# jianzhnie/ScaleRL

Hardware: NVIDIA H100
Metric: learner_frames_per_sec (higher is better)
Workload: dtype bf16

## Files before the change

### scalerl_b200/csrc/encoder.cu

```cuda
#include "encoder_problems.cuh"
#include "tma_problems.cuh"
#include "res_problems.cuh"
#include "enc_fused.cuh"
#include "kernels.h"
#include <stdio.h>
#include <stdlib.h>

namespace srl {

constexpr int PACK_BLOCKS_FK = 256, PACK_BLOCKS_FD = 256, PACK_BLOCKS_CONV = 288;
SRL_DEVINL void pack_store(bf16* __restrict__ out, bf16* __restrict__ out_lo, int64_t i, float v) {
  const bf16 hi = __float2bfloat16_rn(v);
  out[i] = hi;
  if (out_lo) out_lo[i] = __float2bfloat16_rn(v - __bfloat162float(hi));
}
SRL_DEVINL void pack_store2(bf16* __restrict__ out, bf16* __restrict__ out_lo, int64_t i, float v0, float v1) {
  const bf16 h0 = __float2bfloat16_rn(v0), h1 = __float2bfloat16_rn(v1);
  *reinterpret_cast<uint32_t*>(out + i) = pack_bf16x2(v0, v1);
  if (out_lo) *reinterpret_cast<uint32_t*>(out_lo + i) = pack_bf16x2(v0 - __bfloat162float(h0), v1 - __bfloat162float(h1));
}
__global__ void __launch_bounds__(256) pack_weights_kernel(ParamPtrs p, bf16* __restrict__ out, bf16* __restrict__ out_lo, int skip_w1k) {
  pdl_wait(2);
  __shared__ __align__(16) float tile[64 * 99];
  const int t = threadIdx.x, b = blockIdx.x;
  if (b < PACK_BLOCKS_FK) {
    const float4* src = reinterpret_cast<const float4*>(p.wf + (size_t)(2 * b) * 3136);
    float4 v[7];
#pragma unroll
    for (int u = 0; u < 7; ++u) { const int q = t + 256 * u; if (q < 1568) v[u] = __ldg(src + q); }
#pragma unroll
    for (int u = 0; u < 7; ++u) { const int q = t + 256 * u; if (q < 1568) *reinterpret_cast<float4*>(tile + 4 * q) = v[u]; }
    __syncthreads();
#pragma unroll 4
    for (int pp = t; pp < 2 * 1568; pp += 256) {
      const int r = pp >= 1568, k = 2 * (pp - r * 1568), hw = k >> 6, c = k & 63;
      const float* row = tile + r * 3136;
      pack_store2(out, out_lo, WPack::WFK + (int64_t)(2 * b + r) * 3136 + k, row[c * 49 + hw], row[(c + 1) * 49 + hw]);
    }
  } else if (b < PACK_BLOCKS_FK + PACK_BLOCKS_FD) {
    const int bb = b - PACK_BLOCKS_FK, j0 = (bb & 7) * 64, c0 = (bb >> 3) * 2;
    float2 v[13];
#pragma unroll
    for (int u = 0; u < 13; ++u) {
      const int q = t + 256 * u, jj = q / 49, e = q - jj * 49;
      if (q < 64 * 49) v[u] = __ldg(reinterpret_cast<const float2*>(p.wf + (size_t)(j0 + jj) * 3136 + c0 * 49 + 2 * e));
    }
#pragma unroll
    for (int u = 0; u < 13; ++u) {
      const int q = t + 256 * u, jj = q / 49, e = q - jj * 49;
      if (q < 64 * 49) { tile[jj * 99 + 2 * e] = v[u].x; tile[jj * 99 + 2 * e + 1] = v[u].y; }
    }
    __syncthreads();
    const int lane = t & 31, warp = t >> 5;
    for (int kk = warp; kk < 98; kk += 8) {
      const int cc = kk >= 49, hw = kk - cc * 49;
      pack_store2(out, out_lo, WPack::WFD + (int64_t)(hw * 64 + c0 + cc) * 512 + j0 + 2 * lane, tile[(2 * lane) * 99 + kk], tile[(2 * lane + 1) * 99 + kk]);
    }
  } else {
    const int bb = b - PACK_BLOCKS_FK - PACK_BLOCKS_FD;
    constexpr int64_t NCONV = WPack::WFK + (WPack::TOTAL - WPack::W3D);
    for (int64_t n = (int64_t)bb * 256 + t; n < NCONV; n += (int64_t)PACK_BLOCKS_CONV * 256) {
      const int64_t i = n < WPack::WFK ? n : n - WPack::WFK + WPack::W3D;
      float v;
      if (i < WPack::W2K) {
        if (skip_w1k) continue;
        const int e = (int)(i - WPack::W1K), co = e >> 8, k = e & 255, tap = k >> 6, q = k & 63;
        const int c = q >> 4, dy = (q >> 2) & 3, dx = q & 3, kh = 4 * (tap >> 1) + dy, kw = 4 * (tap & 1) + dx;
        v = p.w1[co * 256 + c * 64 + kh * 8 + kw];
      } else if (i < WPack::W3K) {
        const int e = (int)(i - WPack::W2K), co = e >> 9, k = e & 511, tap = k >> 5, c = k & 31;
        v = p.w2[((co * 32 + c) << 4) + tap];
      } else if (i < WPack::WFK) {
        const int e = (int)(i - WPack::W3K), co = e / 576, k = e - co * 576, tap = k >> 6, c = k & 63;
        v = p.w3[(co * 64 + c) * 9 + tap];
      } else if (i < WPack::W2D) {
        const int e = (int)(i - WPack::W3D), c = e / 576, k = e - c * 576, tap = k >> 6, co = k & 63;
        v = p.w3[(co * 64 + c) * 9 + tap];
      } else {
        const int e = (int)(i - WPack::W2D), cls = e >> 13, r = e & 8191, c = r >> 8, k = r & 255, tt = k >> 6, co = k & 63;
        const int kh = (cls >> 1) + 2 * (tt >> 1), kw = (cls & 1) + 2 * (tt & 1);
        v = p.w2[((co * 32 + c) << 4) + kh * 4 + kw];
      }
      pack_store(out, out_lo, i, v);
    }
  }
}

__global__ void __launch_bounds__(352) obs_s2d_kernel(const uint8_t* __restrict__ obs, bf16* __restrict__ xs, int frame_blocks,
                                                      const float* __restrict__ w1, bf16* __restrict__ w1k, bf16* __restrict__ w1k_lo) {
  pdl_wait(1);
  pdl_launch();
  if ((int)blockIdx.x >= frame_blocks) {
    const int e = ((int)blockIdx.x - frame_blocks) * 352 + (int)threadIdx.x;
    if (e < 32 * 256 && w1k) {
      const int co = e >> 8, k = e & 255, tap = k >> 6, q = k & 63;
      const int c = q >> 4, dy = (q >> 2) & 3, dx = q & 3, kh = 4 * (tap >> 1) + dy, kw = 4 * (tap & 1) + dx;
      pack_store(w1k, w1k_lo, e, __ldg(w1 + co * 256 + c * 64 + kh * 8 + kw));
    }
    return;
  }
  __shared__ uint32_t tile[21][16][21];
  const int n = blockIdx.x;
  const int t = threadIdx.x;
  if (t < 336) {
    const int g = t / 21, X = t - g * 21;
    const uint8_t* src = obs + (size_t)n * 28224 + (g >> 2) * 7056 + (g & 3) * 84;
#pragma unroll
    for (int y = 0; y < 21; ++y) tile[y][g][X] = __ldg(reinterpret_cast<const uint32_t*>(src + y * 336) + X);
  }
  __syncthreads();
  if (t < 336) {
    const int X = t >> 4, g = t & 15;
#pragma unroll
    for (int y = 0; y < 21; ++y) {
      const uint32_t w = tile[y][g][X];
      const float f0 = __uint_as_float(__byte_perm(w, 0x4B000000u, 0x7540)) - 8388608.f;
      const float f1 = __uint_as_float(__byte_perm(w, 0x4B000000u, 0x7541)) - 8388608.f;
      const float f2 = __uint_as_float(__byte_perm(w, 0x4B000000u, 0x7542)) - 8388608.f;
      const float f3 = __uint_as_float(__byte_perm(w, 0x4B000000u, 0x7543)) - 8388608.f;
      *reinterpret_cast<uint2*>(xs + (((size_t)n * 21 + y) * 21 + X) * 64 + g * 4) = make_uint2(pack_bf16x2(f0, f1), pack_bf16x2(f2, f3));
    }
  }
}

__global__ void __launch_bounds__(256) a3_transpose_kernel(const bf16* __restrict__ a3, bf16* __restrict__ a3t) {
  pdl_wait(53);
  __shared__ __align__(16) uint16_t tile[49 * 66];
  const int n = blockIdx.x, t = threadIdx.x;
  const uint4* src = reinterpret_cast<const uint4*>(a3 + (size_t)n * 3136);
  for (int q = t; q < 392; q += 256) {
    const uint4 v = __ldg(src + q);
    uint32_t* d = reinterpret_cast<uint32_t*>(tile + (q >> 3) * 66 + (q & 7) * 8);
    d[0] = v.x; d[1] = v.y; d[2] = v.z; d[3] = v.w;
  }
  __syncthreads();
  uint32_t* dst = reinterpret_cast<uint32_t*>(a3t + (size_t)n * 3136);
  for (int pp = t; pp < 1568; pp += 256) {
    const int o = 2 * pp, c0 = o / 49, h0 = o - c0 * 49, o1 = o + 1, c1 = o1 / 49, h1 = o1 - c1 * 49;
    dst[pp] = (uint32_t)tile[h0 * 66 + c0] | ((uint32_t)tile[h1 * 66 + c1] << 16);
  }
}
SRL_KSTAMP_SETTER(kstamp_set_encoder)

cudaError_t launch_a3_transpose(const bf16* a3, bf16* a3t, int frames, cudaStream_t st) {
  if (frames <= 0) return cudaSuccess;
  a3_transpose_kernel<<<frames, 256, 0, st>>>(a3, a3t);
  return cudaGetLastError();
}

cudaError_t launch_pack_weights(const ParamPtrs& p, bf16* wpack, cudaStream_t st, bf16* wpack_lo, bool skip_w1k) {
  pack_weights_kernel<<<PACK_BLOCKS_FK + PACK_BLOCKS_FD + PACK_BLOCKS_CONV, 256, 0, st>>>(p, wpack, wpack_lo, skip_w1k ? 1 : 0);
  return cudaGetLastError();
}

#define SRL_TRY(x) do { cudaError_t e_ = (x); if (e_ != cudaSuccess) return e_; } while (0)

static inline int cdiv(int a, int b) { return (a + b - 1) / b; }

typedef CUresult (*EncodeTiledFn)(CUtensorMap*, CUtensorMapDataType, cuuint32_t, void*, const cuuint64_t*, const cuuint64_t*,
                                  const cuuint32_t*, const cuuint32_t*, CUtensorMapInterleave, CUtensorMapSwizzle,
                                  CUtensorMapL2promotion, CUtensorMapFloatOOBfill);

static EncodeTiledFn encode_fn() {
  static EncodeTiledFn fn = nullptr;
  if (!fn) {
    void* f = nullptr;
    cudaDriverEntryPointQueryResult q;
    if (cudaGetDriverEntryPoint("cuTensorMapEncodeTiled", &f, cudaEnableDefault, &q) == cudaSuccess && q == cudaDriverEntryPointSuccess)
      fn = reinterpret_cast<EncodeTiledFn>(f);
  }
  return fn;
}

bool make_map(CUtensorMap* m, const void* base, int rank, const uint64_t* dims, const uint64_t* strides_elems, const uint32_t* box,
              bool swizzle64) {
  EncodeTiledFn fn = encode_fn();
  if (!fn) return false;
  cuuint64_t gd[5], gs[4];
  cuuint32_t bx[5], es[5];
  for (int i = 0; i < rank; ++i) { gd[i] = dims[i]; bx[i] = box[i]; es[i] = 1; }
  for (int i = 0; i + 1 < rank; ++i) gs[i] = strides_elems[i] * 2;
  return fn(m, CU_TENSOR_MAP_DATA_TYPE_BFLOAT16, (cuuint32_t)rank, const_cast<void*>(base), gd, gs, bx, es, CU_TENSOR_MAP_INTERLEAVE_NONE,
            swizzle64 ? CU_TENSOR_MAP_SWIZZLE_64B : CU_TENSOR_MAP_SWIZZLE_128B, CU_TENSOR_MAP_L2_PROMOTION_L2_128B,
            CU_TENSOR_MAP_FLOAT_OOB_FILL_NONE) == CUDA_SUCCESS;
}

struct MapBuilder {
  const char* failed = nullptr;
  bool lo = false, failed_lo = false;
  void operator()(CUtensorMap* m, const void* base, uint64_t inner, uint64_t rows, uint32_t box_inner, uint32_t box_rows, const char* name,
                  bool swizzle64 = false) {
    const uint64_t d[2] = {inner, rows}, s[1] = {inner};
    const uint32_t bx[2] = {box_inner, box_rows};
    if (!failed && !make_map(m, base, 2, d, s, bx, swizzle64)) { failed = name; failed_lo = lo; }
  }
};

static void build_operand_maps(MapBuilder& mk, const OperandTensors& b, uint64_t nf, uint64_t nb, OperandMaps* M) {
  mk(&M->a1p0_w, b.a1, 64, nf * 100, 64, RConv2Fwd::WROWS, "a1p0_w");
  mk(&M->a1p1_w, b.a1 + (size_t)nf * 100 * 64, 64, nf * 100, 64, RConv2Fwd::WROWS, "a1p1_w");
  mk(&M->a2_w, b.a2, 64, nf * 81, 64, RConv3Fwd::WROWS, "a2_w");
  mk(&M->da3g_w, b.da3, 64, nb * 81, 64, RConv3Dgrad::WROWS, "da3g_w");
  mk(&M->da3g_b, b.da3, 64, nb * 81, 64, 128, "da3g_b");
  mk(&M->da2g_w, b.da2, 64, nb * 100, 64, RConv2Dgrad::WROWS, "da2g_w");
  mk(&M->da2g_b, b.da2, 64, nb * 100, 64, 128, "da2g_b");
  mk(&M->da1g_b, b.da1, 32, nb * 441, 32, 128, "da1g_b", true);
  mk(&M->a3m128, b.a3, 3136, nf, 64, 128, "a3m128");
  mk(&M->a3m64, b.a3, 3136, nf, 64, 64, "a3m64");
  mk(&M->dhm128, b.dh, 512, nb, 64, 128, "dhm128");
  mk(&M->dhm64, b.dh, 512, nb, 64, 64, "dhm64");
  const bf16* w = b.wpack;
  mk(&M->w1k, w + WPack::W1K, 256, 32, 64, 32, "w1k");
  mk(&M->w2k, w + WPack::W2K, 512, 64, 64, 64, "w2k");
  mk(&M->w3k, w + WPack::W3K, 576, 64, 64, 64, "w3k");
  mk(&M->wfk, w + WPack::WFK, 3136, 512, 64, 64, "wfk");
  mk(&M->wfd, w + WPack::WFD, 512, 3136, 64, 64, "wfd");
  mk(&M->w3d, w + WPack::W3D, 576, 64, 64, 64, "w3d");
  mk(&M->w2d, w + WPack::W2D, 256, 128, 64, 128, "w2d");
}

cudaError_t build_tma_maps(const EncoderBuffers& b, int NF, int NB, TmaMaps* M, const char** why) {
  static_assert(RConv1Wgrad::WROWS == RConv1Fwd::WROWS && RConv2Wgrad::WROWS == RConv2Fwd::WROWS && RConv3Wgrad::WROWS == RConv3Fwd::WROWS,
                "forward and wgrad share the window maps");
  const uint64_t nf = NF, nb = NB;
  MapBuilder mk;
  mk(&M->xs_w, b.xs, 64, nf * 441, 64, RConv1Fwd::WROWS, "xs_w");
  mk(&M->a3tm64, b.a3t, 3136, nf, 64, 64, "a3tm64");
  build_operand_maps(mk, b.hi, nf, nb, &M->hi);
  mk.lo = true;
  if (b.lo.wpack) build_operand_maps(mk, b.lo, nf, nb, &M->lo);
  M->valid = !mk.failed;
  if (mk.failed && why) {
    static thread_local char name[32];
    snprintf(name, sizeof(name), "%s%s", mk.failed, mk.failed_lo ? "_lo" : "");
    *why = name;
  }
  return mk.failed ? cudaErrorInvalidValue : cudaSuccess;
}

static cudaError_t launch_s2d(const uint8_t* obs, int frames, bf16* xs, cudaStream_t st, const float* w1, bf16* w1k, bf16* w1k_lo) {
  constexpr int WB = (32 * 256 + 351) / 352;
  SRL_TRY(launch_chain(obs_s2d_kernel, dim3(frames + WB), dim3(352), 0, st, obs, xs, frames, w1, w1k, w1k_lo));
  return cudaGetLastError();
}

static int sm_count() {
  static const int n = [] { int d = 0, v = 0; cudaGetDevice(&d); cudaDeviceGetAttribute(&v, cudaDevAttrMultiProcessorCount, d); return v > 0 ? v : 132; }();
  return n;
}
static int persistent_ctas() {
  static int v = 0;
  if (!v) {
    const char* e = getenv("SRL_PERSISTENT_CTAS");
    v = e ? atoi(e) : sm_count();
    if (v < 16 || v > sm_count()) v = sm_count();
  }
  return v;
}
#define kPersistentCtas persistent_ctas()
static int bwd_ctas() {
  static const int v = [] { const char* e = getenv("SRL_BWD_CTAS"); int x = e ? atoi(e) : 0; return x < 16 || x > sm_count() ? 0 : x; }();
  return v ? v : persistent_ctas() - persistent_ctas() / 9;
}
static int side_wgrad_ctas() {
  static const int v = [] { const char* e = getenv("SRL_WGRAD_CTAS"); int x = e ? atoi(e) : 64; return x < 8 || x > sm_count() ? 64 : x; }();
  return v;
}

struct WgradReduce3 {
  static constexpr int KID = 0, CO = 64, BIAS = 64, PART = WSP_W3, NR = 18, ROW_GROUPS = 32;
  static constexpr bool FRAMES_U8 = false;
  SRL_DEVINL static int row(int rg, int i) { return (i % 9) * 64 + 2 * rg + i / 9; }
};
struct WgradReduce2 {
  static constexpr int KID = 0, CO = 64, BIAS = 64, PART = WSP_W2, NR = 16, ROW_GROUPS = 32;
  static constexpr bool FRAMES_U8 = false;
  SRL_DEVINL static int row(int rg, int i) { return (i >> 2) * 128 + (i & 3) * 32 + rg; }
};
struct WgradReduce1 {
  static constexpr int KID = 51, CO = 32, BIAS = 32, PART = WSP_W1, NR = 16, ROW_GROUPS = 16;
  static constexpr bool FRAMES_U8 = true;
  SRL_DEVINL static int row(int rg, int i) {
    const int c = rg >> 2, kh2 = (rg >> 1) & 1, dy = 2 * (rg & 1) + (i >> 3), kw = i & 7;
    return kh2 * 128 + (kw >> 2) * 64 + c * 16 + dy * 4 + (kw & 3);
  }
};
template <class L>
__global__ void __launch_bounds__(L::NR * 8) conv_wgrad_reduce_kernel(const float* __restrict__ part, int n, float* __restrict__ g,
                                                                       float* __restrict__ db) {
  constexpr int CG = L::CO / 8, TILES = L::ROW_GROUPS * CG;
  static_assert(L::BIAS <= 8 * L::NR, "the bias block fits the tile's threads and shared memory");
  extern __shared__ __align__(16) float stage[];
  pdl_wait(L::KID);
  pdl_launch();
  const int t = threadIdx.x, rg = blockIdx.x / CG, co0 = (blockIdx.x % CG) * 8;
  const bool bias = blockIdx.x == TILES;
  const int per = bias ? L::BIAS / 4 : 2 * L::NR;
  for (int k = t; k < n * per; k += L::NR * 8) {
    const int c = k / per, q = k - c * per;
    const float* src = part + (size_t)c * L::PART + (bias ? L::PART - L::BIAS + 4 * q : L::row(rg, q >> 1) * L::CO + co0 + 4 * (q & 1));
    asm volatile("cp.async.cg.shared.global [%0], [%1], 16;" ::"r"(smem_u32(stage + 4 * k)), "l"(src) : "memory");
  }
  asm volatile("cp.async.wait_all;" ::: "memory");
  __syncthreads();
  const int w = bias ? L::BIAS : 8 * L::NR;
  if (t >= w) return;
  float s = 0.f;
  for (int c = 0; c < n; ++c) s += stage[c * w + t];
  if (bias) db[t] += s;
  else g[(size_t)(co0 + (t & 7)) * (L::ROW_GROUPS * L::NR) + L::NR * rg + (t >> 3)] = L::FRAMES_U8 ? s * (1.0f / 255.0f) : s;
}

template <class L>
static cudaError_t launch_wgrad_reduce(const float* part, int n, float* g, float* db, cudaStream_t st) {
  static PerDeviceOnce once;
  SRL_TRY(ensure_max_dynamic_smem(once, conv_wgrad_reduce_kernel<L>, WG_PART_CTAS * L::NR * 32));
  static const int greatest = [] { int lo = 0, hi = 0; return cudaDeviceGetStreamPriorityRange(&lo, &hi) == cudaSuccess ? hi : 0; }();
  cudaLaunchConfig_t cfg = {};
  cfg.gridDim = dim3(L::ROW_GROUPS * (L::CO / 8) + 1); cfg.blockDim = dim3(L::NR * 8); cfg.dynamicSmemBytes = (size_t)n * L::NR * 32; cfg.stream = st;
  cudaLaunchAttribute attr[1];
  attr[0].id = cudaLaunchAttributePriority;
  attr[0].val.priority = greatest;
  cfg.attrs = attr; cfg.numAttrs = 1;
  return cudaLaunchKernelEx(&cfg, conv_wgrad_reduce_kernel<L>, part, n, g, db);
}

cudaError_t encoder_forward(const uint8_t* obs, int frames, const ParamPtrs& p, const EncoderBuffers& buf, const TmaMaps& maps, int mode,
                            const StepStreams& S, bool fused_front) {
  if (frames <= 0) return cudaSuccess;
  if ((mode != 0 && mode != 1) || !maps.valid) return cudaErrorInvalidValue;
  const int sp = mode;
  if (sp && !buf.lo.wpack) return cudaErrorInvalidValue;
  const cudaStream_t st = S.main;
  if (fused_front && !sp && (reinterpret_cast<uintptr_t>(obs) & 15) == 0) {
    EncFusedParams q{obs, p.w1, p.b1, p.w2, p.b2, buf.xs, buf.hi.a1, buf.hi.a2, frames, buf.NF};
    S.b(PS_ENC_FUSED); SRL_TRY(enc_fused_fwd_launch(q, kPersistentCtas, st)); S.e(PS_ENC_FUSED);
    SRL_TRY(S.join(LANE_PACK));
  } else {
  S.b(PS_S2D); SRL_TRY(launch_s2d(obs, frames, buf.xs, st, p.w1, buf.hi.wpack + WPack::W1K, sp ? buf.lo.wpack + WPack::W1K : nullptr)); S.e(PS_S2D);
  { RConv1Fwd::Params q{maps.xs_w, maps.hi.w1k, maps.lo.w1k, p.b1, buf.hi.a1, buf.lo.a1, frames, buf.NF};
    S.b(PS_CONV1_FWD); SRL_TRY(res_fwd_launch<RConv1Fwd>(q, cdiv(frames * 441, 128), kPersistentCtas, st, sp)); S.e(PS_CONV1_FWD); }
  SRL_TRY(S.join(LANE_PACK));
  { RConv2Fwd::Params q{maps.hi.a1p0_w, maps.hi.a1p1_w, maps.hi.w2k, maps.lo.a1p0_w, maps.lo.a1p1_w, maps.lo.w2k, p.b2, buf.hi.a2, buf.lo.a2, frames};
    S.b(PS_CONV2_FWD); SRL_TRY(res_fwd_launch<RConv2Fwd>(q, cdiv(frames * 100, 128), kPersistentCtas, st, sp)); S.e(PS_CONV2_FWD); }
  }
  { RConv3Fwd::Params q{maps.hi.a2_w, maps.hi.w3k, maps.lo.a2_w, maps.lo.w3k, p.b3, buf.hi.a3, buf.lo.a3, frames};
    S.b(PS_CONV3_FWD); SRL_TRY(res_fwd_launch<RConv3Fwd>(q, cdiv(frames * 81, 128), kPersistentCtas, st, sp)); S.e(PS_CONV3_FWD); }
  { TFcFwd::Params q{maps.hi.a3m128, maps.hi.wfk, maps.lo.a3m128, maps.lo.wfk, buf.hpart, frames};
    static_assert(TFcFwd::SPLITS == FC_SPLITS, "split count");
    S.b(PS_FC_FWD);
    if (sp) SRL_TRY((igemm_tma_launch<TFcFwd, 1>(q, dim3(cdiv(frames, 128), 8 * FC_SPLITS), st)));
    else SRL_TRY((igemm_tma_launch<TFcFwd, 0>(q, dim3(cdiv(frames, 128), 8 * FC_SPLITS), st)));
    S.e(PS_FC_FWD); }
  return cudaSuccess;
}

cudaError_t encoder_backward(int frames, const EncoderBuffers& buf, const ParamPtrs& g, const TmaMaps& maps, int mode,
                             const StepStreams& S, BwdParts parts, bool a3t_done) {
  if (frames <= 0) return cudaSuccess;
  if ((mode != 0 && mode != 1) || !maps.valid) return cudaErrorInvalidValue;
  const int sp = mode;
  if (sp && !buf.lo.wpack) return cudaErrorInvalidValue;
  const bool do_fc = parts & BWD_FC, do_conv = parts & BWD_CONV;
  const cudaStream_t st = S.main, s1 = S.lane(LANE_FC_WGRAD), s2 = S.lane(LANE_CONV3_WGRAD), s3 = S.lane(LANE_CONV2_WGRAD);
  if (do_fc) {
    SRL_TRY(S.fork(LANE_FC_WGRAD));
    { const bool native = !sp && buf.a3t != nullptr;
      S.b(PS_FC_WGRAD);
      if (native) {
        if (!a3t_done) SRL_TRY(launch_a3_transpose(buf.hi.a3, buf.a3t, frames, s1));
        TFcWgradN::Params q{maps.hi.dhm64, maps.a3tm64, g.wf, g.bf, frames};
        SRL_TRY((igemm_tma_launch<TFcWgradN, 0>(q, dim3(1, 4 * (TFcWgradN::NCT + 1)), s1)));
      } else {
        TFcWgrad::Params q{maps.hi.dhm64, maps.hi.a3m64, maps.lo.dhm64, maps.lo.a3m64, g.wf, g.bf, frames};
        if (sp) SRL_TRY((igemm_tma_launch<TFcWgrad, 1>(q, dim3(1, 4 * 50), s1))); else SRL_TRY((igemm_tma_launch<TFcWgrad, 0>(q, dim3(1, 4 * 50), s1)));
      }
      S.e(PS_FC_WGRAD); }
    { TFcDgrad::Params q{maps.hi.dhm128, maps.hi.wfd, maps.lo.dhm128, maps.lo.wfd, buf.hi.a3, buf.hi.da3, buf.lo.da3, frames};
      S.b(PS_FC_DGRAD);
      if (sp) SRL_TRY((igemm_tma_launch<TFcDgrad, 1>(q, dim3(cdiv(frames, 128), 49), st))); else SRL_TRY((igemm_tma_launch<TFcDgrad, 0>(q, dim3(cdiv(frames, 128), 49), st)));
      S.e(PS_FC_DGRAD); }
    if (!do_conv) SRL_TRY(S.join(LANE_FC_WGRAD));
  }
  if (!do_conv) return cudaSuccess;
  SRL_TRY(S.fork(LANE_CONV3_WGRAD));
  float* part3 = buf.wgrad_part;
  float* part2 = part3 + (size_t)WG_PART_CTAS * WSP_W3;
  float* part1 = part2 + (size_t)WG_PART_CTAS * WSP_W2;
  int n3 = 0, n2 = 0, n1 = 0;
  { RConv3Wgrad::Params q{maps.hi.a2_w, maps.hi.da3g_b, maps.lo.a2_w, maps.lo.da3g_b, part3, frames * 81, 0};
    S.b(PS_CONV3_WGRAD); SRL_TRY(res_wgrad_launch<RConv3Wgrad>(q, side_wgrad_ctas(), s2, &n3, sp)); S.e(PS_CONV3_WGRAD); }
  if (!S.collapsed) SRL_TRY(launch_wgrad_reduce<WgradReduce3>(part3, n3, g.w3, g.b3, s2));
  { RConv3Dgrad::Params q{maps.hi.da3g_w, maps.hi.w3d, maps.lo.da3g_w, maps.lo.w3d, buf.hi.a2, buf.hi.da2, buf.lo.da2, frames};
    S.b(PS_CONV3_DGRAD); SRL_TRY(res_fwd_launch<RConv3Dgrad>(q, cdiv(frames * 81, 128), bwd_ctas(), st, sp)); S.e(PS_CONV3_DGRAD); }
  SRL_TRY(S.fork(LANE_CONV2_WGRAD));
  { RConv2Wgrad::Params q{maps.hi.a1p0_w, maps.hi.a1p1_w, maps.hi.da2g_b, maps.lo.a1p0_w, maps.lo.a1p1_w, maps.lo.da2g_b, part2, frames * 100, 0};
    S.b(PS_CONV2_WGRAD); SRL_TRY(res_wgrad_launch<RConv2Wgrad>(q, side_wgrad_ctas(), s3, &n2, sp)); S.e(PS_CONV2_WGRAD); }
  if (!S.collapsed) SRL_TRY(launch_wgrad_reduce<WgradReduce2>(part2, n2, g.w2, g.b2, s3));
  { RConv2Dgrad::Params q{maps.hi.da2g_w, maps.hi.w2d, maps.lo.da2g_w, maps.lo.w2d, buf.hi.a1, buf.hi.da1, buf.lo.da1, frames, buf.NF};
    S.b(PS_CONV2_DGRAD); SRL_TRY(res_fwd_launch<RConv2Dgrad>(q, cdiv(frames * 100, 128), bwd_ctas(), st, sp)); S.e(PS_CONV2_DGRAD); }
  { RConv1Wgrad::Params q{maps.xs_w, maps.hi.da1g_b, maps.lo.da1g_b, part1, frames * 441, 0};
    S.b(PS_CONV1_WGRAD); SRL_TRY(res_wgrad_launch<RConv1Wgrad>(q, bwd_ctas(), st, &n1, sp)); S.e(PS_CONV1_WGRAD); }
  S.b(PS_WGRAD_FINALIZE);
  if (S.collapsed) {
    SRL_TRY(launch_wgrad_reduce<WgradReduce3>(part3, n3, g.w3, g.b3, st));
    SRL_TRY(launch_wgrad_reduce<WgradReduce2>(part2, n2, g.w2, g.b2, st));
  }
  SRL_TRY(launch_wgrad_reduce<WgradReduce1>(part1, n1, g.w1, g.b1, st));
  S.e(PS_WGRAD_FINALIZE);
  if (do_fc) SRL_TRY(S.join(LANE_FC_WGRAD));
  SRL_TRY(S.join(LANE_CONV3_WGRAD));
  SRL_TRY(S.join(LANE_CONV2_WGRAD));
  return cudaSuccess;
}

}
```

### scalerl_b200/csrc/igemm_tma.cuh

```cuda
#pragma once
#include <cuda.h>
#include "common.cuh"
#include "kernels.h"

namespace srl {

SRL_DEVINL void tma_prefetch_desc(const CUtensorMap* m) {
  asm volatile("prefetch.tensormap [%0];" ::"l"(reinterpret_cast<uint64_t>(m)) : "memory");
}
SRL_DEVINL void tma_load_2d(void* dst, const CUtensorMap* m, uint64_t* bar, int c0, int c1) {
  asm volatile("cp.async.bulk.tensor.2d.shared::cluster.global.mbarrier::complete_tx::bytes [%0], [%1, {%3, %4}], [%2];"
               ::"r"(smem_u32(dst)), "l"(reinterpret_cast<uint64_t>(m)), "r"(smem_u32(bar)), "r"(c0), "r"(c1) : "memory");
}
SRL_DEVINL void tma_load_3d(void* dst, const CUtensorMap* m, uint64_t* bar, int c0, int c1, int c2) {
  asm volatile("cp.async.bulk.tensor.3d.shared::cluster.global.mbarrier::complete_tx::bytes [%0], [%1, {%3, %4, %5}], [%2];"
               ::"r"(smem_u32(dst)), "l"(reinterpret_cast<uint64_t>(m)), "r"(smem_u32(bar)), "r"(c0), "r"(c1), "r"(c2) : "memory");
}
SRL_DEVINL void tma_load_4d(void* dst, const CUtensorMap* m, uint64_t* bar, int c0, int c1, int c2, int c3) {
  asm volatile("cp.async.bulk.tensor.4d.shared::cluster.global.mbarrier::complete_tx::bytes [%0], [%1, {%3, %4, %5, %6}], [%2];"
               ::"r"(smem_u32(dst)), "l"(reinterpret_cast<uint64_t>(m)), "r"(smem_u32(bar)), "r"(c0), "r"(c1), "r"(c2), "r"(c3)
               : "memory");
}
SRL_DEVINL void tma_load_5d(void* dst, const CUtensorMap* m, uint64_t* bar, int c0, int c1, int c2, int c3, int c4) {
  asm volatile("cp.async.bulk.tensor.5d.shared::cluster.global.mbarrier::complete_tx::bytes [%0], [%1, {%3, %4, %5, %6, %7}], [%2];"
               ::"r"(smem_u32(dst)), "l"(reinterpret_cast<uint64_t>(m)), "r"(smem_u32(bar)), "r"(c0), "r"(c1), "r"(c2), "r"(c3), "r"(c4)
               : "memory");
}

constexpr int IGT_THREADS = 288;

template <class P, int SPLIT = 0>
struct TmaCfg {
  static constexpr int KROWS = P::A_MN ? P::KROWS : 64;
  static constexpr int A_BYTES = P::A_MN ? 2 * KROWS * 128 : 128 * 128;
  static constexpr int B_BLOCKS = (P::BN + 63) / 64;
  static constexpr int B_BYTES = P::B_MN ? B_BLOCKS * KROWS * 128 : P::BN * 128;
  static constexpr int HALF_BYTES = A_BYTES + B_BYTES;
  static constexpr int STAGE_BYTES = HALF_BYTES * (1 + SPLIT);
  static constexpr int NB = P::BN / 2;
  static constexpr int STAGES = fit_stages(P::STAGES, 2 * WG_IMG_BYTES + 1024 + 256, STAGE_BYTES);
  static constexpr int SMEM_BYTES = STAGES * STAGE_BYTES + 2 * WG_IMG_BYTES + 1024 + 256;
  static_assert(SMEM_BYTES <= 232448, "shared memory budget (227 KB)");
  static_assert(NB == 32 || NB == 64 || NB == 128, "MMA N per warpgroup");
  static constexpr int MMAS = P::A_MN ? KROWS / 16 : 4;
  static_assert(A_BYTES % 1024 == 0 && B_BYTES % 1024 == 0, "operand tiles must keep 1024 B alignment (SWIZZLE_128B atoms)");
  static_assert(P::A_MN == P::B_MN, "mixed majors are not used");
  static_assert(KROWS % 16 == 0, "contraction rows per stage must be a multiple of MMA K = 16");
};

template <class P, int SPLIT>
SRL_DEVINL void igt_epilogue(const typename P::Params& p, int tm, int ty, int row, int c0, float (&v)[16]) {
  if constexpr (SPLIT) P::template epilogue16<1>(p, tm, ty, row, c0, v); else P::epilogue16(p, tm, ty, row, c0, v);
}
template <class P, int SPLIT>
SRL_DEVINL void igt_epilogue(const typename P::Params& p, int tm, int ty, int row, int c0, float (&v)[16], const uint4 (&pre)[2]) {
  if constexpr (SPLIT) P::template epilogue16<1>(p, tm, ty, row, c0, v, pre); else P::epilogue16(p, tm, ty, row, c0, v, pre);
}

template <class P, int SPLIT = 0>
__global__ void __launch_bounds__(IGT_THREADS) igemm_tma_kernel(const __grid_constant__ typename P::Params p) {
  using C = TmaCfg<P, SPLIT>;
  extern __shared__ uint8_t smem_raw[];
  uint8_t* smem = reinterpret_cast<uint8_t*>((reinterpret_cast<uintptr_t>(smem_raw) + 1023) & ~uintptr_t(1023));
  float* img = reinterpret_cast<float*>(smem + C::STAGES * C::STAGE_BYTES);
  uint64_t* bars = reinterpret_cast<uint64_t*>(smem + C::STAGES * C::STAGE_BYTES + 2 * WG_IMG_BYTES);
  uint64_t* full = bars;
  uint64_t* empty = bars + C::STAGES;

  const int tid = threadIdx.x;
  const int warp = tid >> 5;
  const int tm = blockIdx.x, ty = blockIdx.y;
  const int nkb = P::num_kblocks(p, tm, ty);

  if constexpr (P::ZERO_INIT) {
    if (P::zero_cta(ty)) {
      uint4* z = reinterpret_cast<uint4*>(smem);
      for (int i = tid; i < C::STAGES * C::STAGE_BYTES / 16; i += IGT_THREADS) z[i] = make_uint4(0, 0, 0, 0);
    }
    __syncthreads();
    for (int s = 0; s < C::STAGES; ++s) P::init_smem(p, tm, ty, smem + s * C::STAGE_BYTES, tid);
    fence_proxy_async_smem();
  }
  if (warp == 8 && (tid & 31) == 0) {
    for (int s = 0; s < C::STAGES; ++s) { mbar_init(&full[s], 1); mbar_init(&empty[s], 8); }
    mbar_fence_init();
    P::prefetch(p);
  }
  __syncthreads();
  pdl_wait(P::KID);
  if (tid == 256) pdl_launch();

  if (warp == 8) {
    const uint32_t leader = elect_one_sync();
    for (int kb = 0; kb < nkb; ++kb) {
      const int s = kb % C::STAGES;
      mbar_wait(&empty[s], ((kb / C::STAGES) & 1) ^ 1);
      if (leader) {
        uint8_t* sA = smem + s * C::STAGE_BYTES;
        if constexpr (SPLIT) P::issue_split(p, tm, ty, kb, sA, C::A_BYTES, C::HALF_BYTES, &full[s]);
        else P::issue(p, tm, ty, kb, sA, sA + C::A_BYTES, &full[s]);
      }
      __syncwarp();
    }
  } else {
    const int g = warp >> 2, wt = tid & 127;
    constexpr int NB = C::NB;
    uint4 pre[P::PREFETCH ? NB / 16 : 1][2];
    if constexpr (P::PREFETCH) {
#pragma unroll
      for (int c = 0; c < NB / 16; ++c) P::prefetch16(p, tm, ty, wt, g * NB + c * 16, pre[c]);
    }
    float acc[2][NB / 2];
#pragma unroll
    for (int h = 0; h < 2; ++h)
#pragma unroll
      for (int i = 0; i < NB / 2; ++i) acc[h][i] = 0.f;
    constexpr uint32_t ASTEP = P::A_MN ? 2048 / 16 : 32 / 16, BSTEP = P::B_MN ? 2048 / 16 : 32 / 16;
    constexpr uint32_t A_HI = (P::A_MN ? C::KROWS * 128 : 64 * 128) / 16;
    const uint32_t b_off = P::B_MN ? (g * NB / 64) * C::KROWS * 128 + (g * NB % 64) * 2 : g * NB * 128;
    for (int kb = 0; kb < nkb; ++kb) {
      const int s = kb % C::STAGES;
      mbar_wait(&full[s], (kb / C::STAGES) & 1);
      const uint32_t a0 = smem_u32(smem + s * C::STAGE_BYTES);
      const uint64_t ad0 = P::A_MN ? make_smem_desc(a0, C::KROWS * 128, 1024) : make_smem_desc(a0, 16, 1024);
      const uint64_t bd0 = P::B_MN ? make_smem_desc(a0 + C::A_BYTES + b_off, C::KROWS * 128, 1024) : make_smem_desc(a0 + C::A_BYTES + b_off, 16, 1024);
      wg_fence();
#pragma unroll
      for (int k = 0; k < C::MMAS; ++k) {
        const uint64_t ad = ad0 + (uint64_t)(k * ASTEP), bd = bd0 + (uint64_t)(k * BSTEP);
        wg_mma128<NB, P::A_MN ? 1 : 0, P::B_MN ? 1 : 0>(acc, ad, A_HI, bd, (kb | k) != 0);
        if constexpr (SPLIT) {
          wg_mma128<NB, P::A_MN ? 1 : 0, P::B_MN ? 1 : 0>(acc, ad, A_HI, bd + (uint64_t)(C::HALF_BYTES / 16), 1);
          wg_mma128<NB, P::A_MN ? 1 : 0, P::B_MN ? 1 : 0>(acc, ad + (uint64_t)(C::HALF_BYTES / 16), A_HI, bd, 1);
        }
      }
      wg_commit();
      if constexpr (C::STAGES > 1) {
        wg_wait_prev();
        __syncwarp();
        if (kb > 0 && (tid & 31) == 0) mbar_arrive(&empty[(kb - 1) % C::STAGES]);
      } else {
        wg_wait_all();
        __syncwarp();
        if ((tid & 31) == 0) mbar_arrive(&empty[s]);
      }
    }
    wg_wait_all();
    wg_fence_regs(acc[0]); wg_fence_regs(acc[1]);
    float* my_img = img + g * (WG_IMG_BYTES / 4);
#pragma unroll
    for (int c = 0; c < NB / 16; ++c) {
      float v[16];
      wg_acc_row16<NB>(acc, c, my_img, wt, 2 + g, v);
      if constexpr (P::PREFETCH) igt_epilogue<P, SPLIT>(p, tm, ty, wt, g * NB + c * 16, v, pre[c]);
      else igt_epilogue<P, SPLIT>(p, tm, ty, wt, g * NB + c * 16, v);
    }
  }
}

template <class P, int SPLIT = 0>
cudaError_t igemm_tma_launch(const typename P::Params& p, dim3 grid, cudaStream_t stream) {
  using C = TmaCfg<P, SPLIT>;
  if (grid.x == 0 || grid.y == 0) return cudaSuccess;
  static PerDeviceOnce once;
  { cudaError_t e = ensure_max_dynamic_smem(once, igemm_tma_kernel<P, SPLIT>, C::SMEM_BYTES); if (e != cudaSuccess) return e; }
  return launch_chain(igemm_tma_kernel<P, SPLIT>, grid, dim3(IGT_THREADS), C::SMEM_BYTES, stream, p);
}

}
```

### scalerl_b200/csrc/tma_problems.cuh

```cuda
#pragma once
#include "igemm_tma.cuh"
#include "encoder_problems.cuh"

namespace srl {

#define SRL_TMAP alignas(64) CUtensorMap

struct TFcFwd {
  static constexpr int KID = 31;
  static constexpr bool PREFETCH = false;
  static constexpr int BN = 64, STAGES = 4, SPLITS = 4;
  static constexpr bool A_MN = false, B_MN = false, ZERO_INIT = false;
  static constexpr int KROWS = 64;
  struct Params { SRL_TMAP a3m; SRL_TMAP w; SRL_TMAP a3m_lo; SRL_TMAP w_lo; float* out; int M; };
  SRL_DEVINL static void prefetch(const Params& p) { tma_prefetch_desc(&p.a3m); tma_prefetch_desc(&p.w); }
  SRL_DEVINL static int kb_begin(int split) { return (49 * split) / SPLITS; }
  SRL_DEVINL static void issue_split(const Params& p, int tm, int ty, int kb, uint8_t* st, int a_bytes, int half, uint64_t* bar) {
    const int k = (kb_begin(ty % SPLITS) + kb) * 64;
    mbar_arrive_expect_tx(bar, 2 * (128 * 128 + 64 * 128));
    tma_load_2d(st, &p.a3m, bar, k, tm * 128);
    tma_load_2d(st + a_bytes, &p.w, bar, k, (ty / SPLITS) * 64);
    tma_load_2d(st + half, &p.a3m_lo, bar, k, tm * 128);
    tma_load_2d(st + half + a_bytes, &p.w_lo, bar, k, (ty / SPLITS) * 64);
  }
  template <int SPLIT>
  SRL_DEVINL static void epilogue16(const Params& p, int tm, int ty, int row, int c0, float (&v)[16]) { epilogue16(p, tm, ty, row, c0, v); }
  SRL_DEVINL static int num_kblocks(const Params&, int, int ty) { const int sp = ty % SPLITS; return kb_begin(sp + 1) - kb_begin(sp); }
  SRL_DEVINL static void issue(const Params& p, int tm, int ty, int kb, uint8_t* sA, uint8_t* sB, uint64_t* bar) {
    const int k = (kb_begin(ty % SPLITS) + kb) * 64;
    mbar_arrive_expect_tx(bar, 128 * 128 + 64 * 128);
    tma_load_2d(sA, &p.a3m, bar, k, tm * 128);
    tma_load_2d(sB, &p.w, bar, k, (ty / SPLITS) * 64);
  }
  SRL_DEVINL static void epilogue16(const Params& p, int tm, int ty, int row, int c0, float (&v)[16]) {
    const int m = tm * 128 + row;
    if (m >= p.M) return;
    float4* o = reinterpret_cast<float4*>(p.out + ((size_t)(ty % SPLITS) * p.M + m) * 512 + (ty / SPLITS) * 64 + c0);
#pragma unroll
    for (int j = 0; j < 4; ++j) o[j] = make_float4(v[4 * j], v[4 * j + 1], v[4 * j + 2], v[4 * j + 3]);
  }
};

struct TFcDgrad {
  static constexpr int KID = 32;
  static constexpr bool PREFETCH = true;
  static constexpr int BN = 64, STAGES = 4;
  static constexpr bool A_MN = false, B_MN = false, ZERO_INIT = false;
  static constexpr int KROWS = 64;
  struct Params { SRL_TMAP dhm; SRL_TMAP w; SRL_TMAP dhm_lo; SRL_TMAP w_lo; const bf16* a3; bf16* da3; bf16* da3_lo; int M; };
  SRL_DEVINL static void prefetch(const Params& p) { tma_prefetch_desc(&p.dhm); tma_prefetch_desc(&p.w); }
  SRL_DEVINL static int num_kblocks(const Params&, int, int) { return 8; }
  SRL_DEVINL static void issue_split(const Params& p, int tm, int ty, int kb, uint8_t* st, int a_bytes, int half, uint64_t* bar) {
    mbar_arrive_expect_tx(bar, 2 * (128 * 128 + 64 * 128));
    tma_load_2d(st, &p.dhm, bar, kb * 64, tm * 128);
    tma_load_2d(st + a_bytes, &p.w, bar, kb * 64, ty * 64);
    tma_load_2d(st + half, &p.dhm_lo, bar, kb * 64, tm * 128);
    tma_load_2d(st + half + a_bytes, &p.w_lo, bar, kb * 64, ty * 64);
  }
  SRL_DEVINL static void issue(const Params& p, int tm, int ty, int kb, uint8_t* sA, uint8_t* sB, uint64_t* bar) {
    mbar_arrive_expect_tx(bar, 128 * 128 + 64 * 128);
    tma_load_2d(sA, &p.dhm, bar, kb * 64, tm * 128);
    tma_load_2d(sB, &p.w, bar, kb * 64, ty * 64);
  }
  SRL_DEVINL static void prefetch16(const Params& p, int tm, int ty, int row, int c0, uint4 (&mk)[2]) {
    const int m = tm * 128 + row;
    if (m < p.M) ld_mask16(p.a3 + (size_t)m * 3136 + ty * 64 + c0, mk);
  }
  SRL_DEVINL static void epilogue16(const Params& p, int tm, int ty, int row, int c0, float (&v)[16], const uint4 (&mk)[2]) {
    epilogue16<0>(p, tm, ty, row, c0, v, mk);
  }
  template <int SPLIT>
  SRL_DEVINL static void epilogue16(const Params& p, int tm, int ty, int row, int c0, float (&v)[16], const uint4 (&mk)[2]) {
    const int m = tm * 128 + row;
    if (m >= p.M) return;
    relu_mask16_pre(mk, v);
    const size_t o = ((size_t)m * 81 + (ty / 7) * 9 + ty % 7) * 64 + c0;
    store_bf16x16(p.da3 + o, v);
    if constexpr (SPLIT) {
      float r[16];
#pragma unroll
      for (int j = 0; j < 16; ++j) r[j] = v[j] - __bfloat162float(__float2bfloat16_rn(v[j]));
      store_bf16x16(p.da3_lo + o, r);
    }
  }
};

SRL_DEVINL void fill_ones(uint8_t* dst, int bytes, int tid) {
  uint4* q = reinterpret_cast<uint4*>(dst);
  for (int i = tid; i < bytes / 16; i += IGT_THREADS) q[i] = make_uint4(0x3F803F80u, 0x3F803F80u, 0x3F803F80u, 0x3F803F80u);
}

struct TFcWgrad {
  static constexpr int KID = 33;
  static constexpr bool PREFETCH = false;
  static constexpr int BN = 64, STAGES = 4, KROWS = 64;
  static constexpr bool A_MN = true, B_MN = true, ZERO_INIT = true;
  struct Params { SRL_TMAP dhm; SRL_TMAP a3m; SRL_TMAP dhm_lo; SRL_TMAP a3m_lo; float* dw; float* db; int M; };
  SRL_DEVINL static void prefetch(const Params& p) { tma_prefetch_desc(&p.dhm); tma_prefetch_desc(&p.a3m); }
  SRL_DEVINL static void issue_split(const Params& p, int, int ty, int kb, uint8_t* st, int a_bytes, int half, uint64_t* bar) {
    const int hw = ty >> 2, j0 = (ty & 3) * 128;
    mbar_arrive_expect_tx(bar, (hw < 49 ? 6 : 4) * 64 * 128);
    tma_load_2d(st, &p.dhm, bar, j0, kb * 64);
    tma_load_2d(st + KROWS * 128, &p.dhm, bar, j0 + 64, kb * 64);
    tma_load_2d(st + half, &p.dhm_lo, bar, j0, kb * 64);
    tma_load_2d(st + half + KROWS * 128, &p.dhm_lo, bar, j0 + 64, kb * 64);
    if (hw < 49) {
      tma_load_2d(st + a_bytes, &p.a3m, bar, hw * 64, kb * 64);
      tma_load_2d(st + half + a_bytes, &p.a3m_lo, bar, hw * 64, kb * 64);
    }
  }
  template <int SPLIT>
  SRL_DEVINL static void epilogue16(const Params& p, int tm, int ty, int row, int c0, float (&v)[16]) { epilogue16(p, tm, ty, row, c0, v); }
  SRL_DEVINL static bool zero_cta(int) { return true; }
  SRL_DEVINL static int num_kblocks(const Params& p, int, int) { return (p.M + 63) >> 6; }
  SRL_DEVINL static void init_smem(const Params&, int, int ty, uint8_t* stage, int tid) {
    if ((ty >> 2) == 49) fill_ones(stage + 2 * KROWS * 128, KROWS * 128, tid);
  }
  SRL_DEVINL static void issue(const Params& p, int, int ty, int kb, uint8_t* sA, uint8_t* sB, uint64_t* bar) {
    const int hw = ty >> 2, j0 = (ty & 3) * 128;
    mbar_arrive_expect_tx(bar, (hw < 49 ? 3 : 2) * 64 * 128);
    tma_load_2d(sA, &p.dhm, bar, j0, kb * 64);
    tma_load_2d(sA + KROWS * 128, &p.dhm, bar, j0 + 64, kb * 64);
    if (hw < 49) tma_load_2d(sB, &p.a3m, bar, hw * 64, kb * 64);
  }
  SRL_DEVINL static void epilogue16(const Params& p, int, int ty, int row, int c0, float (&v)[16]) {
    const int j = (ty & 3) * 128 + row, hw = ty >> 2;
    if (hw < 49) {
#pragma unroll
      for (int jj = 0; jj < 16; ++jj) p.dw[(size_t)j * 3136 + (c0 + jj) * 49 + hw] = v[jj];
    } else if (c0 == 0) {
      p.db[j] = v[0];
    }
  }
};

struct TFcWgradN {
  static constexpr int KID = 36;
  static constexpr bool PREFETCH = false;
  static constexpr int BN = 256, STAGES = 4, KROWS = 64, NCT = 13;
  static constexpr bool A_MN = true, B_MN = true, ZERO_INIT = true;
  struct Params { SRL_TMAP dhm; SRL_TMAP a3tm; float* dw; float* db; int M; };
  SRL_DEVINL static void prefetch(const Params& p) { tma_prefetch_desc(&p.dhm); tma_prefetch_desc(&p.a3tm); }
  SRL_DEVINL static bool zero_cta(int ty) { return (ty >> 2) == NCT; }
  SRL_DEVINL static int num_kblocks(const Params& p, int, int) { return (p.M + 63) >> 6; }
  SRL_DEVINL static void init_smem(const Params&, int, int ty, uint8_t* stage, int tid) {
    if ((ty >> 2) == NCT) fill_ones(stage + 2 * KROWS * 128, KROWS * 128, tid);
  }
  SRL_DEVINL static void issue(const Params& p, int, int ty, int kb, uint8_t* sA, uint8_t* sB, uint64_t* bar) {
    const int ct = ty >> 2, j0 = (ty & 3) * 128;
    const int nb = ct < NCT ? (ct == NCT - 1 ? 1 : 4) : 0;
    mbar_arrive_expect_tx(bar, (2 + nb) * 64 * 128);
    tma_load_2d(sA, &p.dhm, bar, j0, kb * 64);
    tma_load_2d(sA + KROWS * 128, &p.dhm, bar, j0 + 64, kb * 64);
    for (int q = 0; q < nb; ++q) tma_load_2d(sB + q * KROWS * 128, &p.a3tm, bar, ct * 256 + q * 64, kb * 64);
  }
  SRL_DEVINL static void epilogue16(const Params& p, int, int ty, int row, int c0, float (&v)[16]) {
    const int j = (ty & 3) * 128 + row, ct = ty >> 2, col = ct * 256 + c0;
    if (ct < NCT) {
      if (col < 3136) {
        float4* d = reinterpret_cast<float4*>(p.dw + (size_t)j * 3136 + col);
#pragma unroll
        for (int q = 0; q < 4; ++q) d[q] = make_float4(v[4 * q], v[4 * q + 1], v[4 * q + 2], v[4 * q + 3]);
      }
    } else if (c0 == 0) {
      p.db[j] = v[0];
    }
  }
};

}
```

Baseline: 2.506 million.

## Widen FC dgrad tiles to 128 columns and stage FC wgrad epilogue through ring smem

The FC dgrad GEMM goes from 64-wide to 128-wide N tiles, so its grid drops from 49 to 25 column tiles. Each CTA loads two weight blocks per k-step, giving more reuse of the dhm A-tile, and the last tile is masked. The native FC wgrad epilogue now writes accumulators into the reused operand ring as an fp32 tile. It then stores rows to global as coalesced float4s instead of per-warpgroup image staging, which frees the image smem. This adds extra named barriers and per-element bounds checks, and fewer CTAs may lower occupancy or wave balance.

After: 2.497 million, median of 6. About the same (-0.4%).

```diff
diff --git a/scalerl_b200/csrc/encoder.cu b/scalerl_b200/csrc/encoder.cu
--- a/scalerl_b200/csrc/encoder.cu
+++ b/scalerl_b200/csrc/encoder.cu
@@ -378,7 +378,8 @@
       S.e(PS_FC_WGRAD); }
     { TFcDgrad::Params q{maps.hi.dhm128, maps.hi.wfd, maps.lo.dhm128, maps.lo.wfd, buf.hi.a3, buf.hi.da3, buf.lo.da3, frames};
       S.b(PS_FC_DGRAD);
-      if (sp) SRL_TRY((igemm_tma_launch<TFcDgrad, 1>(q, dim3(cdiv(frames, 128), 49), st))); else SRL_TRY((igemm_tma_launch<TFcDgrad, 0>(q, dim3(cdiv(frames, 128), 49), st)));
+      const dim3 grid(cdiv(frames, 128), TFcDgrad::NCT);
+      if (sp) SRL_TRY((igemm_tma_launch<TFcDgrad, 1>(q, grid, st))); else SRL_TRY((igemm_tma_launch<TFcDgrad, 0>(q, grid, st)));
       S.e(PS_FC_DGRAD); }
     if (!do_conv) SRL_TRY(S.join(LANE_FC_WGRAD));
   }
diff --git a/scalerl_b200/csrc/igemm_tma.cuh b/scalerl_b200/csrc/igemm_tma.cuh
--- a/scalerl_b200/csrc/igemm_tma.cuh
+++ b/scalerl_b200/csrc/igemm_tma.cuh
@@ -1,5 +1,6 @@
 #pragma once
 #include <cuda.h>
+#include <type_traits>
 #include "common.cuh"
 #include "kernels.h"
 
@@ -29,6 +30,21 @@
 
 constexpr int IGT_THREADS = 288;
 
+template <class P, class = void> struct RingPitch { static constexpr int value = 0; };
+template <class P> struct RingPitch<P, std::void_t<decltype(P::RING_PITCH)>> { static constexpr int value = P::RING_PITCH; };
+
+template <int N, int PITCH>
+SRL_DEVINL void wg_acc_stage_f32(const float (&d)[2][N / 2], float* buf, int wt) {
+  const int w = wt >> 5, l = wt & 31;
+#pragma unroll
+  for (int h = 0; h < 2; ++h)
+#pragma unroll
+    for (int i = 0; i < N / 2; i += 2) {
+      const int row = 64 * h + 16 * w + (l >> 2) + 8 * ((i >> 1) & 1), col = 8 * (i >> 2) + 2 * (l & 3);
+      *reinterpret_cast<float2*>(buf + row * PITCH + col) = make_float2(d[h][i], d[h][i + 1]);
+    }
+}
+
 template <class P, int SPLIT = 0>
 struct TmaCfg {
   static constexpr int KROWS = P::A_MN ? P::KROWS : 64;
@@ -38,9 +54,12 @@
   static constexpr int HALF_BYTES = A_BYTES + B_BYTES;
   static constexpr int STAGE_BYTES = HALF_BYTES * (1 + SPLIT);
   static constexpr int NB = P::BN / 2;
-  static constexpr int STAGES = fit_stages(P::STAGES, 2 * WG_IMG_BYTES + 1024 + 256, STAGE_BYTES);
-  static constexpr int SMEM_BYTES = STAGES * STAGE_BYTES + 2 * WG_IMG_BYTES + 1024 + 256;
+  static constexpr bool RING_EPI = RingPitch<P>::value > 0 && !SPLIT;
+  static constexpr int IMG_BYTES = RING_EPI ? 0 : WG_IMG_BYTES;
+  static constexpr int STAGES = fit_stages(P::STAGES, 2 * IMG_BYTES + 1024 + 256, STAGE_BYTES);
+  static constexpr int SMEM_BYTES = STAGES * STAGE_BYTES + 2 * IMG_BYTES + 1024 + 256;
   static_assert(SMEM_BYTES <= 232448, "shared memory budget (227 KB)");
+  static_assert(!RING_EPI || 128 * RingPitch<P>::value * 4 <= STAGES * STAGE_BYTES, "the fp32 tile fits the operand ring");
   static_assert(NB == 32 || NB == 64 || NB == 128, "MMA N per warpgroup");
   static constexpr int MMAS = P::A_MN ? KROWS / 16 : 4;
   static_assert(A_BYTES % 1024 == 0 && B_BYTES % 1024 == 0, "operand tiles must keep 1024 B alignment (SWIZZLE_128B atoms)");
@@ -63,7 +82,7 @@
   extern __shared__ uint8_t smem_raw[];
   uint8_t* smem = reinterpret_cast<uint8_t*>((reinterpret_cast<uintptr_t>(smem_raw) + 1023) & ~uintptr_t(1023));
   float* img = reinterpret_cast<float*>(smem + C::STAGES * C::STAGE_BYTES);
-  uint64_t* bars = reinterpret_cast<uint64_t*>(smem + C::STAGES * C::STAGE_BYTES + 2 * WG_IMG_BYTES);
+  uint64_t* bars = reinterpret_cast<uint64_t*>(smem + C::STAGES * C::STAGE_BYTES + 2 * C::IMG_BYTES);
   uint64_t* full = bars;
   uint64_t* empty = bars + C::STAGES;
 
@@ -147,13 +166,22 @@
     }
     wg_wait_all();
     wg_fence_regs(acc[0]); wg_fence_regs(acc[1]);
-    float* my_img = img + g * (WG_IMG_BYTES / 4);
+    if constexpr (C::RING_EPI) {
+      constexpr int PITCH = RingPitch<P>::value;
+      float* tile = reinterpret_cast<float*>(smem);
+      named_bar(1, 256);
+      wg_acc_stage_f32<NB, PITCH>(acc, tile + g * NB, wt);
+      named_bar(1, 256);
+      P::epilogue_rows(p, tm, ty, tid, tile);
+    } else {
+      float* my_img = img + g * (WG_IMG_BYTES / 4);
 #pragma unroll
-    for (int c = 0; c < NB / 16; ++c) {
-      float v[16];
-      wg_acc_row16<NB>(acc, c, my_img, wt, 2 + g, v);
-      if constexpr (P::PREFETCH) igt_epilogue<P, SPLIT>(p, tm, ty, wt, g * NB + c * 16, v, pre[c]);
-      else igt_epilogue<P, SPLIT>(p, tm, ty, wt, g * NB + c * 16, v);
+      for (int c = 0; c < NB / 16; ++c) {
+        float v[16];
+        wg_acc_row16<NB>(acc, c, my_img, wt, 2 + g, v);
+        if constexpr (P::PREFETCH) igt_epilogue<P, SPLIT>(p, tm, ty, wt, g * NB + c * 16, v, pre[c]);
+        else igt_epilogue<P, SPLIT>(p, tm, ty, wt, g * NB + c * 16, v);
+      }
     }
   }
 }
diff --git a/scalerl_b200/csrc/tma_problems.cuh b/scalerl_b200/csrc/tma_problems.cuh
--- a/scalerl_b200/csrc/tma_problems.cuh
+++ b/scalerl_b200/csrc/tma_problems.cuh
@@ -44,37 +44,42 @@
 struct TFcDgrad {
   static constexpr int KID = 32;
   static constexpr bool PREFETCH = true;
-  static constexpr int BN = 64, STAGES = 4;
+  static constexpr int BN = 128, STAGES = 4, NCT = 25;
   static constexpr bool A_MN = false, B_MN = false, ZERO_INIT = false;
   static constexpr int KROWS = 64;
   struct Params { SRL_TMAP dhm; SRL_TMAP w; SRL_TMAP dhm_lo; SRL_TMAP w_lo; const bf16* a3; bf16* da3; bf16* da3_lo; int M; };
   SRL_DEVINL static void prefetch(const Params& p) { tma_prefetch_desc(&p.dhm); tma_prefetch_desc(&p.w); }
   SRL_DEVINL static int num_kblocks(const Params&, int, int) { return 8; }
+  SRL_DEVINL static int w_blocks(int ty) { return ty == NCT - 1 ? 1 : 2; }
   SRL_DEVINL static void issue_split(const Params& p, int tm, int ty, int kb, uint8_t* st, int a_bytes, int half, uint64_t* bar) {
-    mbar_arrive_expect_tx(bar, 2 * (128 * 128 + 64 * 128));
+    const int nb = w_blocks(ty);
+    mbar_arrive_expect_tx(bar, 2 * (128 * 128 + nb * 64 * 128));
     tma_load_2d(st, &p.dhm, bar, kb * 64, tm * 128);
-    tma_load_2d(st + a_bytes, &p.w, bar, kb * 64, ty * 64);
     tma_load_2d(st + half, &p.dhm_lo, bar, kb * 64, tm * 128);
-    tma_load_2d(st + half + a_bytes, &p.w_lo, bar, kb * 64, ty * 64);
+    for (int q = 0; q < nb; ++q) {
+      tma_load_2d(st + a_bytes + q * 64 * 128, &p.w, bar, kb * 64, ty * 128 + q * 64);
+      tma_load_2d(st + half + a_bytes + q * 64 * 128, &p.w_lo, bar, kb * 64, ty * 128 + q * 64);
+    }
   }
   SRL_DEVINL static void issue(const Params& p, int tm, int ty, int kb, uint8_t* sA, uint8_t* sB, uint64_t* bar) {
-    mbar_arrive_expect_tx(bar, 128 * 128 + 64 * 128);
+    const int nb = w_blocks(ty);
+    mbar_arrive_expect_tx(bar, 128 * 128 + nb * 64 * 128);
     tma_load_2d(sA, &p.dhm, bar, kb * 64, tm * 128);
-    tma_load_2d(sB, &p.w, bar, kb * 64, ty * 64);
+    for (int q = 0; q < nb; ++q) tma_load_2d(sB + q * 64 * 128, &p.w, bar, kb * 64, ty * 128 + q * 64);
   }
   SRL_DEVINL static void prefetch16(const Params& p, int tm, int ty, int row, int c0, uint4 (&mk)[2]) {
     const int m = tm * 128 + row;
-    if (m < p.M) ld_mask16(p.a3 + (size_t)m * 3136 + ty * 64 + c0, mk);
+    if (m < p.M && 2 * ty + (c0 >> 6) < 49) ld_mask16(p.a3 + (size_t)m * 3136 + ty * 128 + c0, mk);
   }
   SRL_DEVINL static void epilogue16(const Params& p, int tm, int ty, int row, int c0, float (&v)[16], const uint4 (&mk)[2]) {
     epilogue16<0>(p, tm, ty, row, c0, v, mk);
   }
   template <int SPLIT>
   SRL_DEVINL static void epilogue16(const Params& p, int tm, int ty, int row, int c0, float (&v)[16], const uint4 (&mk)[2]) {
-    const int m = tm * 128 + row;
-    if (m >= p.M) return;
+    const int m = tm * 128 + row, hw = 2 * ty + (c0 >> 6);
+    if (m >= p.M || hw >= 49) return;
     relu_mask16_pre(mk, v);
-    const size_t o = ((size_t)m * 81 + (ty / 7) * 9 + ty % 7) * 64 + c0;
+    const size_t o = ((size_t)m * 81 + (hw / 7) * 9 + hw % 7) * 64 + (c0 & 63);
     store_bf16x16(p.da3 + o, v);
     if constexpr (SPLIT) {
       float r[16];
@@ -154,16 +159,19 @@
     tma_load_2d(sA + KROWS * 128, &p.dhm, bar, j0 + 64, kb * 64);
     for (int q = 0; q < nb; ++q) tma_load_2d(sB + q * KROWS * 128, &p.a3tm, bar, ct * 256 + q * 64, kb * 64);
   }
-  SRL_DEVINL static void epilogue16(const Params& p, int, int ty, int row, int c0, float (&v)[16]) {
-    const int j = (ty & 3) * 128 + row, ct = ty >> 2, col = ct * 256 + c0;
-    if (ct < NCT) {
-      if (col < 3136) {
-        float4* d = reinterpret_cast<float4*>(p.dw + (size_t)j * 3136 + col);
-#pragma unroll
-        for (int q = 0; q < 4; ++q) d[q] = make_float4(v[4 * q], v[4 * q + 1], v[4 * q + 2], v[4 * q + 3]);
-      }
-    } else if (c0 == 0) {
-      p.db[j] = v[0];
+  static constexpr int RING_PITCH = 256 + 8;
+  SRL_DEVINL static void epilogue_rows(const Params& p, int, int ty, int t, const float* tile) {
+    const int j0 = (ty & 3) * 128, ct = ty >> 2;
+    if (ct == NCT) {
+      if (t < 128) p.db[j0 + t] = tile[t * RING_PITCH];
+      return;
+    }
+    const int nk = ct == NCT - 1 ? 16 : 64;
+#pragma unroll 8
+    for (int s = 0; s < 32; ++s) {
+      const int e = s * 256 + t, r = e >> 6, k = e & 63;
+      if (k < nk)
+        *reinterpret_cast<float4*>(p.dw + (size_t)(j0 + r) * 3136 + ct * 256 + 4 * k) = *reinterpret_cast<const float4*>(tile + r * RING_PITCH + 4 * k);
     }
   }
 };
```
